# TimoLassmann/tagdust

Measured on AMD Instinct MI355X. Metric: reads/s (150 bp, 8-barcode arch), higher is better.
Workload: dtype f32

## Files before the change

tagdust_amd/csrc/td_jit.h:

```cpp
#pragma once
#include <string>
#include <vector>
#include "../../include/tagdust_hip.h"
#include "td_device.h"

#ifndef TD_HIDDEN
#define TD_HIDDEN __attribute__((visibility("hidden")))
#endif

struct TdSpecKnobs {
	int block = 512;
	int min_waves = 4;
	int lsum_oob = 1;
	int rt_min = 16;
	int groupcols = 18;
	int groupcols_fwd = 12;
	int prune = 1;
	int prune_sfx = 1;
	int restart = -1;
	int firstseg = -1;
	int trie_sh = 2;
	int profile = 0;
	int prune_stats = -1;
	std::string extra_opts;
};
TdSpecKnobs td_spec_knobs(void);

#define TD_PRUNE_TABLES 16
#define TD_PRUNE_RESTART_MAX 4

struct TdSpecPlan {
	TdSpecKnobs k;
	int S = 0, H = 0, C = 0;
	std::vector<int> col_off, hmm_off;
	std::vector<int> group, group_f;
	std::vector<int> pure_last, drop_m;
	std::vector<int> bw_off;
	int64_t halves = 0;
	std::vector<int> rt, rt_b;
	std::vector<int> base;
	std::vector<float> hi, lo, nv;
	bool trie_on = false;
	int trie_sh = 1, trie_n_share = 0;
	std::vector<int> trie_ord;
	int first_n = 0;
	int prune_segs = 0;
	int sfx_first = 0;
	float prune_z = 0.0f;
	int restart = 0;
};
TdSpecPlan td_spec_plan(const td_model_desc* m, const TdSpecKnobs& k);
TD_HIDDEN std::string td_spec_model_section(const td_model_desc* m, const TdSpecPlan& p, int lsum_oob, int window);

float td_spec_prune_z(const td_model_desc* m, int n_seg, int sfx_first);
void td_spec_prune_tables(const td_model_desc* m, const TdSpecPlan& p, int lcap, int stride, std::vector<float>& tab);
void td_spec_layout(TdSpecLayout& L, const TdSpecPlan& p, int lmax);
int td_spec_compile(const td_model_desc* m, const TdSpecPlan& p, int lsum_oob, int window, std::vector<char>& code, std::string& log,
                    uint64_t* key_out = nullptr, bool key_only = false);
int td_spec_compiles_started(void);
```

tagdust_amd/csrc/td_spec_kernel.inc:

```

#ifndef TDS_BLOCK
#define TDS_BLOCK 512
#endif
#ifndef TDS_MIN_WAVES
#define TDS_MIN_WAVES 4
#endif
#define TDS_REG_H 32
#define TDS_WPB (TDS_BLOCK / TD_WAVE)
#define NEG_INF (-__builtin_inff())
#define DEV __device__ __forceinline__

#define MODE_GET_LABEL 1
#define MODE_ARCH_COMP 5
#define OUT_SUCCESS 0
#define OUT_ARCH_MISMATCH 1
#define OUT_TOO_SHORT 2
#define OUT_BAR_FINGER_NOT_FOUND 3
#define OUT_MATCHES_ARTIFACTS 5
#define OUT_LOW_COMPLEXITY 6
#define N_OUTCOME_SLOTS 8
#define TDS_DIAG(k) (N_OUTCOME_SLOTS + 256 + ((k) - 192))

#ifndef TDS_LSUM_OOB
#define TDS_LSUM_OOB 1
// ... 127 lines not shown
DEV float emit_rt(const int b, const float hi, const float lo, const float nv, const BaseMask& k, const int x)
{
	const float r = (x == b) ? hi : lo;
	return k.m4 ? nv : r;
}

#ifndef TDS_PROFILE
#define TDS_PROFILE 0
#endif
#define TDS_PHASE(k) do { if (TDS_PROFILE) { const long long t_ = (long long)__builtin_readcyclecounter(); \
	if (lane == 0) atomicAdd(&ka.counters[TDS_DIAG(240 + (k))], (unsigned long long)(t_ - tprof)); tprof = t_; } } while (0)

#ifndef TDS_WINDOW
#define TDS_WINDOW 0
#endif
constexpr bool kMaskDP = TD_H - kFirstN <= TDS_REG_H;

struct Wv {
	uint32_t* pmask;
	int nwm;
	uint8_t* slot;
	int lane, len, lmax, tmax, tmin;
	float* bm;
	uint8_t* ba;
	int cut;
	int cutS;
	const float* wa;
	const float* wb;
	int sstop;
	int sstopS;
	const float* wc;
	const float* wd;
	mutable int bad;
	bool rb_on, rf_on;
	float* rs;
	float* hb;
	int rWf;
	int rW;
	const float* bwt;
	const float* fbs;
	unsigned long long* stats;
	long long* tprof;
	const float* ptab;
	int pstride;
	const float* qr;
	const float* pr;
};

#ifndef TDS_LATE_CS
#define TDS_LATE_CS 1
#endif
#ifndef TDS_PF_DIST
#define TDS_PF_DIST 4
#endif
#ifndef TDS_PF_COLS
#define TDS_PF_COLS 2
#endif
#ifndef TDS_LDP
#define TDS_LDP 2
#endif
#ifndef TDS_LDT
#define TDS_LDT 4
#endif
#ifndef TDS_SCAN_B
#define TDS_SCAN_B 8
#endif
#ifndef TDS_PRUNE_TT
#define TDS_PRUNE_TT (-88.0f)
#endif
#ifndef TDS_PRUNE_MARGIN
#define TDS_PRUNE_MARGIN 1
#endif
#ifndef TDS_PRUNE_BGAP
#define TDS_PRUNE_BGAP 5.0f
#endif
#ifndef TDS_PRUNE_STATS
#define TDS_PRUNE_STATS 0
#endif

constexpr int cmin(int a, int b) { return a < b ? a : b; }
constexpr int pf_dist(int cols, bool rt) { return (!rt && cols <= TDS_PF_COLS) ? TDS_PF_DIST : 1; }
template <int D> struct IC { static constexpr int v = D; };
constexpr bool label_leading(int h)
{
	for (int j = 0; j < kPruneSegs; j++) if (h >= kHmmOff[j] && h < kHmmOff[j] + kNHmm[j]) return true;
	return false;
}
template <int PD, int D, typename F>
DEV void ring_block(F& step, const int base)
{
	if constexpr (D < PD) { step(IC<D>{}, base + D); ring_block<PD, D + 1>(step, base); }
}
template <int PD, int D, typename F>
DEV void ring_rest(F& step, const int base, const int iend)
{
	if constexpr (D < PD - 1) { if (base + D <= iend) { step(IC<D>{}, base + D); ring_rest<PD, D + 1>(step, base, iend); } }
}

template <int J, bool RT>
DEV void bwd_row(const int fa, const float (&Mn)[kNCol[J]], const float (&In)[kNCol[J]], const float Pn,
                 const BaseMask& kc, const int c, const BaseMask& kx, const int xi, SV (&Mc)[kNCol[J]], SV (&Ic)[kNCol[J]])
{
#define EM(gcol, mask, xval) (RT ? emit_rt(kBase[colr + (gcol)], kHi[J], kLo[J], kNv[J], mask, xval) : EMIT_M(col0 + (gcol), mask))
	constexpr int NC = kNCol[J];
	constexpr int K = NC - 1;
	const int col0 = kColOff[J] + (RT ? 0 : fa) * NC;
// ... 631 lines not shown
	constexpr int NC = kNCol[J];
	float hi0 = NEG_INF;
	{
		const float* gf = w.ptab + (int64_t)(12 + J - kSfxFirst) * w.pstride;
		const int t = q_lo - 1;
		for (int k0 = 1; k0 <= t; k0 += 8) {
			float pr[8];
#pragma unroll
			for (int u = 0; u < 8; u++) { const int k = k0 + u; pr[u] = w.pr[((k <= t) ? t - k : 0) * TD_WAVE + w.lane]; }
			__builtin_amdgcn_sched_barrier(0);
#pragma unroll
			for (int u = 0; u < 8; u++) { const int k = k0 + u; if (k <= t) hi0 = fmaxf(hi0, uload(gf, k) + pr[u]); }
		}
		hi0 = fminf(hi0 + (__logf((float)(t > 1 ? t : 1)) + 0.02f), w.fbs[t]);
	}
	float Mlo[NC], Mhi[NC], Ilo[NC], Ihi[NC];
#pragma unroll
	for (int g = 0; g < NC; g++) { Mlo[g] = NEG_INF; Ilo[g] = NEG_INF; Mhi[g] = hi0; Ihi[g] = hi0; }
	int gc = 0;
	int closed_at = -1;
	auto close_check = [&](const int steps_done) __attribute__((always_inline)) {
		if (gc < NC) {
			bool cl = true;
#pragma unroll
			for (int g = 0; g < NC; g++) if (g == gc) cl = same(si(Mlo[g], Mhi[g])) && same(si(Ilo[g], Ihi[g]));
			if (__builtin_amdgcn_ballot_w64(!cl) == 0) { gc++; if (gc == NC) closed_at = steps_done; }
		}
	};
	int c_n = codes[q_lo * TD_WAVE + w.lane];
	float Pm_n = P[(q_lo - 1) * TD_WAVE + w.lane];
	for (int i = q_lo; i < q_hi; ++i) {
		const int c = c_n;
		const float Pm = Pm_n;
		{
			const int ip = (i + 1 < q_hi) ? i + 1 : i;
			c_n = codes[ip * TD_WAVE + w.lane];
			Pm_n = P[(ip - 1) * TD_WAVE + w.lane];
		}
		close_check(i - q_lo); close_check(i - q_lo);
		fstair_dispatch<J, 0>(gc, Mlo, Mhi, Ilo, Ihi, Pm, mk_mask(c));
	}
	close_check(q_hi - q_lo); close_check(q_hi - q_lo);
	if (gc < NC) w.bad |= 32;
	if (TDS_PRUNE_STATS && w.lane == 0) {
		const int st = closed_at >= 0 ? closed_at : q_hi - q_lo;
		atomicAdd(&w.stats[TDS_DIAG(194)], (unsigned long long)st); atomicAdd(&w.stats[TDS_DIAG(195)], 1ull);
		atomicMax(&w.stats[TDS_DIAG(192)], (unsigned long long)st);
	}
	float* rs = w.rs + (int64_t)kColOff[J] * 2 * TD_WAVE + w.lane;
#pragma unroll
	for (int g = 0; g < NC; g++) { rs[(2 * g) * TD_WAVE] = Mlo[g]; rs[(2 * g + 1) * TD_WAVE] = Ilo[g]; }
}

template <int J, int NF, bool RT>
DEV void fwd_group(const Wv& w, const uint8_t* __restrict__ codes, const float* __restrict__ P,
                   float* __restrict__ Cs, const float* __restrict__ PB, const uint8_t* __restrict__ BW,
                   float* __restrict__ DP, float* __restrict__ TOTAL, const float b, const int f0)
{
	const bool first = (f0 == 0);
#define EM(gcol, mask, xval) (RT ? emit_rt(kBase[colr + (gcol)], kHi[J], kLo[J], kNv[J], mask, xval) : EMIT_M(col0 + (gcol), mask))
	constexpr int NC = kNCol[J];
	constexpr int K = NC - 1;
	constexpr bool pure = kPureLast[J] != 0;
	constexpr int NS = NC - kPureLast[J];
	constexpr int DM = kDropM[J];
	constexpr int NSF = NS - DM;
	constexpr int ROWH = 2 * NS - DM;
	constexpr int NQ = NSF / 2;
	constexpr int NT = NSF & 1;
	constexpr bool skip_live = LIVE(kSkip[J]);
	float Mp[NF][NC], Ip[NF][NC], tot[NF];
#pragma unroll
	for (int f = 0; f < NF; f++) {
		tot[f] = NEG_INF;
#pragma unroll
		for (int g = 0; g < NC; g++) { Mp[f][g] = NEG_INF; Ip[f][g] = NEG_INF; }
	}
	if (TDS_RESTART && J >= kSfxFirst && w.rf_on) {
		const float* rs = w.rs + (int64_t)kColOff[J] * 2 * TD_WAVE + w.lane;
#pragma unroll
		for (int g = 0; g < NC; g++) { Mp[0][g] = rs[(2 * g) * TD_WAVE]; Ip[0][g] = rs[(2 * g + 1) * TD_WAVE]; }
	}
	constexpr bool p_init = (J == 0);
	const bool resumed = TDS_RESTART && (J >= kSfxFirst) && w.rf_on;
	const int i0 = resumed ? w.sstop - (TD_S - 1 - J) * (w.rWf + 1) : 1;
	float Pm = p_init ? 0.0f : P[(i0 - 1) * TD_WAVE + w.lane];
	constexpr int PD = pf_dist(NF * NC, RT);
	const int pmax = (w.tmax >= 1) ? w.tmax : 1;
	int c_q[PD];
	float Pi_q[PD], cs_q[PD], pb_q[PD], bm_q[PD], ik_q[PD][NF];
	int ba_q[PD];
	float MB_q[PD][NF][NSF + 1], IB_q[PD][NF][NSF + 1];
	constexpr bool pb_init = (J == TD_S - 1);
#define PBR(pos) (pb_init ? (((pos) == w.len + 1) ? 0.0f : NEG_INF) : PB[(pos) * TD_WAVE + w.lane])
#define BWROW(f_, pos_) (BW + ((int64_t)kBwOff[kHmmOff[J] + f0 + (f_)] * w.lmax + (int64_t)((pos_) - 1) * ROWH) * (TD_WAVE * 4))
#define TDS_FWD_FILL(d, p_raw) { \
		const int p_ = ((p_raw) <= pmax) ? (p_raw) : pmax; \
		c_q[d] = codes[p_ * TD_WAVE + w.lane]; \
		Pi_q[d] = p_init ? NEG_INF : P[p_ * TD_WAVE + w.lane]; \
		if (!first) cs_q[d] = Cs[p_ * TD_WAVE + w.lane]; \
		if (pure) pb_q[d] = PBR(p_ + 1); \
		if (own_sum && !first) { bm_q[d] = w.bm[p_ * TD_WAVE + w.lane]; ba_q[d] = w.ba[p_ * TD_WAVE + w.lane]; } \
		const bool rows_ = !((J >= kSfxFirst) && p_ < w.sstop);    \
_Pragma("unroll") \
		for (int f = 0; f < NF; f++) { \
			if (DM && rows_) ik_q[d][f] = ld1(BWROW(f, p_) + NSF * (TD_WAVE * 8), w.lane); \
			if (PD > 1 && rows_) { \
_Pragma("unroll") \
				for (int q = 0; q < NQ; q++) { \
					MB_q[d][f][2 * q] = ldk(BWROW(f, p_) + q * (TD_WAVE * 16), w.lane, 16, 0); IB_q[d][f][2 * q] = ldk(BWROW(f, p_) + q * (TD_WAVE * 16), w.lane, 16, 1); \
					MB_q[d][f][2 * q + 1] = ldk(BWROW(f, p_) + q * (TD_WAVE * 16), w.lane, 16, 2); IB_q[d][f][2 * q + 1] = ldk(BWROW(f, p_) + q * (TD_WAVE * 16), w.lane, 16, 3); \
				} \
				if (NT) { MB_q[d][f][NSF - 1] = ldk(BWROW(f, p_) + NQ * (TD_WAVE * 16), w.lane, 8, 0); IB_q[d][f][NSF - 1] = ldk(BWROW(f, p_) + NQ * (TD_WAVE * 16), w.lane, 8, 1); } \
			} \
		} \
	}
	constexpr bool own_sum = (J == 0) && (kFirstN > 0);
	float lacc[NF];
	uint32_t mbits[NF];
#pragma unroll
	for (int f = 0; f < NF; f++) { lacc[f] = 0.0f; mbits[f] = 0u; }
#pragma unroll
	for (int d = 0; d < PD; d++) {
		cs_q[d] = NEG_INF; pb_q[d] = 0.0f; bm_q[d] = -1.0f; ba_q[d] = 0;
#pragma unroll
		for (int f = 0; f < NF; f++) ik_q[d][f] = NEG_INF;
		TDS_FWD_FILL(d, i0 + d)
	}

	const int iend = (J < kPruneSegs && w.cut < w.tmax) ? w.cut : w.tmax;
	const int itail = (J == kPruneSegs && kPruneSegs > 0) ? w.cut + 1 : w.tmax + 1;
	(void)itail;
	if (i0 > 1 && kMaskDP && !own_sum) {
#pragma unroll
		for (int f = 0; f < NF; f++) {
			if (w.lane == 0) for (int wd = 0; wd < ((i0 - 1) >> 5); wd++) w.pmask[(kHmmOff[J] + f0 + f) * w.nwm + wd] = 0u;
			mbits[f] = 0u;
		}
	}
	auto step_cs = [&](auto dtag, auto cstag, const int i) __attribute__((always_inline)) {
		constexpr int d_ = decltype(dtag)::v;
		constexpr bool want_cs = decltype(cstag)::v != 0;
		const int c = c_q[d_];
		const float Pi = Pi_q[d_];
		const float pb = pb_q[d_];
		SV cs; cs.v = cs_q[d_]; cs.z = RT ? false : first;
		float bm = bm_q[d_];
		int ba = ba_q[d_];
		f32x4 cb[NF][NQ + 1];
		f32x2 ct[NF];
		const bool sfx_skip = (J >= kSfxFirst) && i < w.sstop;
		float ik[NF];
#pragma unroll
		for (int f = 0; f < NF; f++) {
			if constexpr (PD == 1) {
				const uint8_t* bw = BW + ((int64_t)kBwOff[kHmmOff[J] + f0 + f] * w.lmax + (int64_t)(i - 1) * ROWH) * (TD_WAVE * 4);
				if (!sfx_skip) {
#pragma unroll
					for (int p = 0; p < NQ; p++) cb[f][p] = ld4(bw + p * (TD_WAVE * 16), w.lane);
					if (NT) ct[f] = ld2(bw + NQ * (TD_WAVE * 16), w.lane);
				}
			} else {
#pragma unroll
				for (int p = 0; p < NQ; p++) cb[f][p] = f32x4{ MB_q[d_][f][2 * p], IB_q[d_][f][2 * p], MB_q[d_][f][2 * p + 1], IB_q[d_][f][2 * p + 1] };
				if (NT) ct[f] = f32x2{ MB_q[d_][f][NSF - 1], IB_q[d_][f][NSF - 1] };
			}
			ik[f] = ik_q[d_][f];
		}
		TDS_FWD_FILL(d_, i + PD)
		const int dn_ = (d_ + 1) % PD;
		const int c_n = c_q[dn_];
		const float pb_n = pb_q[dn_];
		float ik_n[NF];
#pragma unroll
		for (int f = 0; f < NF; f++) ik_n[f] = ik_q[dn_][f];
		float lpost[NF];
#pragma unroll
		for (int f = 0; f < NF; f++) lpost[f] = NEG_INF;
		const bool tail = (J == kPruneSegs && kPruneSegs > 0) && i >= itail;
		if (i <= w.len) {
			const SV PmS = sv(tail ? NEG_INF : Pm);
			const SV PiS = sv(tail ? NEG_INF : Pi);
			const BaseMask kc = mk_mask(c);
#pragma unroll
			for (int f = 0; f < NF; f++) {
				const int col0 = kColOff[J] + (RT ? 0 : (f0 + f)) * NC;
				const int colr = kColOff[J] + (f0 + f) * NC;
				(void)colr;
				const int h = kHmmOff[J] + f0 + f;
				SV Mc[NC], Ic[NC];
				SV Dc = sv_none();
				const float ei0 = EMIT_I(col0, kc);
				{
					const int q = col0;
					const SV M = addv(addc(PmS, kCols[q].sM), EM(0, kc, c));
					SV I = addc(PmS, kCols[q].sI);
					if (tail && LIVE(kCols[q].sI)) {
						if (!(Ip[f][0] + kCols[q].t[3] >= uload(w.wa, i))) w.bad |= 1;
					}
					I = lsum(I, addc(sv(Ip[f][0]), kCols[q].t[3]));
					I = lsum(I, addc(sv(Mp[f][0]), kCols[q].t[1]));
					I = addv(I, ei0);
					if (want_cs) { cs = lsum(cs, addc(M, kCols[q].t[7])); cs = lsum(cs, addc(I, kCols[q].t[8])); }
					Mc[0] = M; Ic[0] = I;
				}
#pragma unroll
				for (int g = 1; g <= K; ++g) {
					const int q = col0 + g, qp = q - 1;
					SV M = addc(PmS, kCols[q].sM);
					SV I = addc(PmS, kCols[q].sI);
					lsum2(M, addc(sv(Mp[f][g - 1]), kCols[qp].t[0]), I, addc(sv(Ip[f][g]), kCols[q].t[3]));
					lsum2(M, addc(sv(Ip[f][g - 1]), kCols[qp].t[4]), I, addc(sv(Mp[f][g]), kCols[q].t[1]));
					SV D = addc(Mc[g - 1], kCols[qp].t[2]);
					lsum2(M, addc(Dc, kCols[qp].t[6]), D, addc(Dc, kCols[qp].t[5]));
					M = addv(M, EM(g, kc, c));
					I = addv(I, EMIT_I(q, kc));
					if (want_cs) { cs = lsum(cs, addc(M, kCols[q].t[7])); cs = lsum(cs, addc(I, kCols[q].t[8])); }
					Mc[g] = M; Ic[g] = I; Dc = D;
				}
				if (tail && skip_live) { if (!(cs.v >= uload(w.wb, i))) w.bad |= 2; }
				if (want_cs) cs = lsum(cs, addc(PiS, kSkip[J]));
				if (!sfx_skip) {
				float MB[NC], IB[NC];
#pragma unroll
				for (int p = 0; p < NQ; p++) {
					const f32x4 v = cb[f][p];
					MB[2 * p] = v.x; IB[2 * p] = v.y; MB[2 * p + 1] = v.z; IB[2 * p + 1] = v.w;
				}
				if (NT) { MB[NSF - 1] = ct[f].x; IB[NSF - 1] = ct[f].y; }
				if constexpr (DM != 0) {
					constexpr int g = K - 1;
					const int q = col0 + g;
					const bool nxt = i < w.len;
					const int cx = (i < w.tmax) ? c_n : 0;
					const BaseMask kn = mk_mask(cx);
					SV MnK = addc(sv(pb_n), kCols[col0 + K].t[7]);
					if (!MnK.z) MnK.v = nxt ? MnK.v : NEG_INF;
					const float InK = nxt ? ik_n[f] : NEG_INF;
					SV Mr = addc(addv(MnK, EM(K, kn, cx)), kCols[q].t[0]);
					Mr = lsum(Mr, addc(sv(pb), kCols[q].t[7]));
					Mr = lsum(Mr, addc(addv(sv(InK), EMIT_I(q, kn)), kCols[q].t[1]));
					MB[g] = Mr.v; IB[g] = ik[f];
				}
				if (pure) {
					MB[K] = pb + kCols[col0 + K].t[7];
					IB[K] = pb + kCols[col0 + K].t[8];
				}
				constexpr bool want_tt = kNHmm[J] > 1;
				SV acc = sv_none(), tt = sv(tot[f]);
#pragma unroll
				for (int g = 0; g <= K; ++g) {
					const SV pm = subv(addv(Mc[g], MB[g]), b);
					if (want_tt && g == 0) tt = lsum(tt, pm);
					acc = lsum(acc, pm);
					if (want_tt && g == 0) tt = lsum(tt, subv(addv(addv(addc(PmS, kCols[col0].sI), ei0), IB[0]), b));
					acc = lsum(acc, subv(addv(Ic[g], IB[g]), b));
				}
				if (want_tt) tot[f] = tt.v;
				if (own_sum) {
					lacc[f] = post_prob(acc.v) + lacc[f];
					if (lacc[f] > bm) { bm = lacc[f]; ba = h; }
				} else if (kMaskDP) {
					lpost[f] = acc.v;
				} else {
					DP[((int64_t)(i - 1) * TD_H + h) * TD_WAVE + w.lane] = post_prob(acc.v);
				}
				}
#pragma unroll
				for (int g = 0; g < NC; g++) { Mp[f][g] = Mc[g].v; Ip[f][g] = Ic[g].v; }
			}
			if (want_cs) Cs[i * TD_WAVE + w.lane] = cs.v;
			if (own_sum) { w.bm[i * TD_WAVE + w.lane] = bm; w.ba[i * TD_WAVE + w.lane] = (uint8_t)ba; }
		}
		if (kMaskDP && !own_sum) {
#pragma unroll
			for (int f = 0; f < NF; f++) {
				const bool on = lpost[f] > -103.98f;
				const bool any_on = __builtin_amdgcn_ballot_w64(on) != 0;
				if (any_on) {
					float pp = 0.0f;
					if (on) pp = (float)exp((double)lpost[f]);
					if (i <= w.len) DP[((int64_t)(i - 1) * TD_H + kHmmOff[J] + f0 + f) * TD_WAVE + w.lane] = pp;
				}
				mbits[f] |= (any_on ? 1u : 0u) << ((i - 1) & 31);
				if ((((i - 1) & 31) == 31) || i == iend) {
					if (w.lane == 0) w.pmask[(kHmmOff[J] + f0 + f) * w.nwm + ((i - 1) >> 5)] = mbits[f];
					mbits[f] = 0u;
				}
			}
		}
		Pm = Pi;
	};
	{
		constexpr bool cs_late = TDS_LATE_CS && (J == TD_S - 1) && !((J == kPruneSegs && kPruneSegs > 0) && skip_live);
		auto step = [&](auto dtag, const int i) __attribute__((always_inline)) { step_cs(dtag, IC<1>{}, i); };
		auto step_nocs = [&](auto dtag, const int i) __attribute__((always_inline)) { step_cs(dtag, IC<0>{}, i); };
		int base = i0;
		if constexpr (cs_late) {
			const int i_cs = (w.tmin < iend) ? w.tmin : iend;
			for (; base + PD - 1 < i_cs; base += PD) ring_block<PD, 0>(step_nocs, base);
		}
		for (; base + PD - 1 <= iend; base += PD) ring_block<PD, 0>(step, base);
		ring_rest<PD, 0>(step, base, iend);
	}
	if (J < kPruneSegs && iend < w.tmax) {
		if (kMaskDP && !own_sum && w.lane == 0) {
#pragma unroll
			for (int f = 0; f < NF; f++)
				for (int wd = ((iend - 1) >> 5) + 1; wd < w.nwm; wd++) w.pmask[(kHmmOff[J] + f0 + f) * w.nwm + wd] = 0u;
		}
		if (kNHmm[J] > 1 && w.len > iend) {
#pragma unroll
			for (int f = 0; f < NF; f++) if (!(tot[f] >= TDS_PRUNE_TT)) w.bad |= 4;
		}
	}
	if (kNHmm[J] > 1) {
#pragma unroll
		for (int f = 0; f < NF; f++) TOTAL[(kHmmOff[J] + f0 + f) * TD_WAVE + w.lane] = tot[f];
	}
#undef EM
#undef PBR
#undef BWROW
#undef TDS_FWD_FILL
}

template <int J, int F0>
DEV void fwd_groups(const Wv& w, const uint8_t* __restrict__ codes, const float* __restrict__ P,
                    float* __restrict__ Cs, const float* __restrict__ PB, const uint8_t* __restrict__ BW,
                    float* __restrict__ DP, float* __restrict__ TOTAL, const float b)
{
	if constexpr (TDS_RESTART && F0 == 0 && J >= kSfxFirst) {
		if (w.rf_on) {
			const int q_hi = w.sstop - (TD_S - 1 - J) * (w.rWf + 1);
			fwd_stair<J>(w, codes, P, q_hi - w.rWf, q_hi);
		}
	}
	if constexpr (F0 == 0 && kRt[J] > 0) {
		for (int f0 = 0; f0 < kRt[J]; f0 += kGroupF[J]) fwd_group<J, kGroupF[J], true>(w, codes, P, Cs, PB, BW, DP, TOTAL, b, f0);
		fwd_groups<J, kRt[J]>(w, codes, P, Cs, PB, BW, DP, TOTAL, b);
	} else if constexpr (F0 < kNHmm[J]) {
		constexpr int NF = cmin(kGroupF[J], kNHmm[J] - F0);
		fwd_group<J, NF, false>(w, codes, P, Cs, PB, BW, DP, TOTAL, b, F0);
		fwd_groups<J, F0 + NF>(w, codes, P, Cs, PB, BW, DP, TOTAL, b);
	}
}

template <int J>
DEV void fwd_segments(const Wv& w, const uint8_t* __restrict__ codes, float* __restrict__ SF, const float* __restrict__ SB,
                      int rowlen, const uint8_t* __restrict__ BW, float* __restrict__ DP, float* __restrict__ TOTAL, const float b)
{
	if constexpr (J < TD_S) {
		fwd_groups<J, 0>(w, codes, SF + (int64_t)J * rowlen, SF + (int64_t)(J + 1) * rowlen, SB + (int64_t)(J + 1) * rowlen,
		                 BW, DP, TOTAL, b);
		if (TDS_PROFILE == 2 && J < 8) { const long long t_ = (long long)__builtin_readcyclecounter(); if (w.lane == 0) atomicAdd(&w.stats[TDS_DIAG(216 + J)], (unsigned long long)(t_ - *w.tprof)); *w.tprof = t_; }
		fwd_segments<J + 1>(w, codes, SF, SB, rowlen, BW, DP, TOTAL, b);
	}
}

constexpr bool path_word_trivial(int k)
{
	for (int b = 0; b < 4; b++) {
		const int v = kFirstN + 4 * k + b;
		if (v < TD_H && (kPredFirst[v] != 0 || kPredOff2[v + 1] != kPredOff2[v])) return false;
	}
	return true;
}
constexpr uint32_t path_word_identity(int k)
{
	uint32_t w = 0;
	for (int b = 0; b < 4; b++) w |= (uint32_t)((kFirstN + 4 * k + b) & 0xFF) << (8 * b);
	return w;
}

DEV int prune_scan(const float thr, const int len, const int tmax, const float* __restrict__ fbt, const float* __restrict__ bwt)
{
	int cl = 1;
	for (int i0 = 2; i0 <= tmax; i0 += TDS_SCAN_B) {
		float g[TDS_SCAN_B];
#pragma unroll
		for (int k = 0; k < TDS_SCAN_B; k++) {
			const int i = i0 + k;
			const int mm = (i <= len) ? len - i : 0;
			g[k] = bwt[mm];
		}
		__builtin_amdgcn_sched_barrier(0);
#pragma unroll
		for (int k = 0; k < TDS_SCAN_B; k++) g[k] = uload(fbt, i0 + k) + g[k];
#pragma unroll
		for (int k = 0; k < TDS_SCAN_B; k++) {
			const int i = i0 + k;
			if (i <= len && i <= tmax && g[k] > thr) cl = i;
		}
	}
#pragma unroll
	for (int o = 32; o >= 1; o >>= 1) cl = max(cl, __shfl_xor(cl, o));
	return __builtin_amdgcn_readfirstlane(cl);
}

DEV float leading_bwd_bound(const Wv& w, const int i)
{
	float hb = NEG_INF;
	for (int k0 = 0; i + 1 + k0 <= w.tmax + 1; k0 += TDS_SCAN_B) {
		float q[TDS_SCAN_B];
#pragma unroll
		for (int u = 0; u < TDS_SCAN_B; u++) {
// ... 905 lines not shown
```

tagdust_amd/csrc/td_spec_plan.cpp:

```cpp
#include <math.h>
#include <stdio.h>
#include <stdlib.h>
#include <string.h>

#include <map>
#include <string>
#include <vector>

#include "td_jit.h"

static std::string flit(float v)
{
	if (isinf(v)) return v < 0 ? "(-__builtin_inff())" : "__builtin_inff()";
	if (v != v) return "__builtin_nanf(\"\")";
	char buf[64];
	snprintf(buf, sizeof buf, "%af", (double)v);
	return buf;
}

TdSpecKnobs td_spec_knobs(void)
{
	TdSpecKnobs k;
	auto num = [](const char* name, int unset) { const char* e = getenv(name); return e ? atoi(e) : unset; };
	auto flag = [](const char* name, int unset) -> int { const char* e = getenv(name); return e ? atoi(e) != 0 : unset; };
	if (const int v = num("TD_SPEC_BLOCK", 0); v >= 64 && v <= 1024 && v % 64 == 0) k.block = v;
	if (const int v = num("TD_SPEC_MINWAVES", 0); v >= 1 && v <= 8) k.min_waves = v;
	if (const int v = num("TD_SPEC_GROUPCOLS", 0); v > 0) k.groupcols = v;
	k.groupcols_fwd = num("TD_SPEC_GROUPCOLS_FWD", k.groupcols_fwd);
	k.rt_min = num("TD_SPEC_RT_MIN", k.rt_min);
	k.trie_sh = num("TD_SPEC_TRIE_SH", k.trie_sh);
	k.profile = num("TD_SPEC_PROFILE", k.profile);
	k.lsum_oob = flag("TD_SPEC_LSUM_OOB", k.lsum_oob);
	k.prune = flag("TD_SPEC_PRUNE", k.prune);
	k.prune_sfx = flag("TD_SPEC_PRUNE_SFX", k.prune_sfx);
	k.restart = flag("TD_SPEC_RESTART", k.restart);
	k.firstseg = flag("TD_SPEC_FIRSTSEG", k.firstseg);
	k.prune_stats = flag("TD_SPEC_PRUNE_STATS", k.prune_stats);
	if (const char* e = getenv("TD_SPEC_EXTRA_OPTS")) k.extra_opts = e;
	return k;
}

namespace {
int pure_last(const td_model_desc* m, int j, int col_off)
{
	for (int f = 0; f < m->n_hmm[j]; f++) {
		const int q = col_off + f * m->n_col[j] + m->n_col[j] - 1;
		if (!(m->trans[q * 9 + 4] == -INFINITY) || !(m->trans[q * 9 + 3] == -INFINITY)) return 0;
	}
	return 1;
}

int rt_prefix(const td_model_desc* m, int j, int col_off, int* base , float* hi, float* lo, float* nv, int min_hmms)
{
	const int n = m->n_hmm[j], nc = m->n_col[j];
	if (n < min_hmms) return 0;
	auto match_type = [&](int q, int* b, float* h, float* l, float* v) -> bool {
		const float* e = m->eM + (size_t)q * 5;
		for (int x = 0; x < 4; x++) {
			const float other = e[(x + 1) & 3];
			bool ok = !(e[x] == other);
			for (int y = 0; y < 4 && ok; y++) if (y != x && !(e[y] == other)) ok = false;
			if (ok) { *b = x; *h = e[x]; *l = other; *v = e[4]; return true; }
		}
		return false;
	};
	int b0; float h0, l0, v0;
	if (!match_type(col_off, &b0, &h0, &l0, &v0)) return 0;
	int f = 0;
	for (; f < n; f++) {
		bool ok = true;
		for (int g = 0; g < nc && ok; g++) {
			const int q = col_off + f * nc + g, q0 = col_off + g;
			if (memcmp(m->trans + (size_t)q * 9, m->trans + (size_t)q0 * 9, 36) || memcmp(m->eI + (size_t)q * 5, m->eI + (size_t)q0 * 5, 20) ||
			    memcmp(&m->sM[q], &m->sM[q0], 4) || memcmp(&m->sI[q], &m->sI[q0], 4)) { ok = false; break; }
			int b; float h, l, v;
			if (!match_type(q, &b, &h, &l, &v) || memcmp(&h, &h0, 4) || memcmp(&l, &l0, 4) || memcmp(&v, &v0, 4)) { ok = false; break; }
			base[q] = b;
		}
		if (!ok) break;
	}
	*hi = h0; *lo = l0; *nv = v0;
	return f >= min_hmms ? f : 0;
}

int group_size(int n_hmm, int n_col, int target)
{
	int maxf = target / n_col;
	if (maxf < 1) maxf = 1;
	if (maxf > n_hmm) maxf = n_hmm;
	const int groups = (n_hmm + maxf - 1) / maxf;
	return (n_hmm + groups - 1) / groups;
}

int first_labels(const td_model_desc* m, int firstseg)
{
	const int H = m->H, n0 = m->n_hmm[0];
	const int mode = firstseg >= 0 ? firstseg : H > 32;
	if (!mode) return 0;
	if (n0 < 2 || n0 >= H) return 0;
	for (int v = 0; v < n0; v++)
		for (int u = 0; u < v; u++) if (m->A[u * H + v] == 1.0f) return 0;
	for (int w = n0; w < H; w++) {
		int c = 0;
		for (int u = 0; u < n0; u++) c += m->A[u * H + w] == 1.0f;
		if (c != 0 && c != n0) return 0;
	}
	return n0;
}

bool read_like(const td_model_desc* m, int j, int co)
{
	if (m->n_hmm[j] != 1 || m->n_col[j] != 1) return false;
	const float* t = m->trans + (size_t)co * 9;
	for (int k = 0; k < 9; k++) if (k != TD_II && k != TD_ISKIP && t[k] > -INFINITY) return false;
	return m->sM[co] == -INFINITY && m->sI[co] > -INFINITY && t[TD_II] > -INFINITY && t[TD_ISKIP] > -INFINITY;
}
}

TdSpecPlan td_spec_plan(const td_model_desc* m, const TdSpecKnobs& k)
{
	TdSpecPlan p;
	const int S = m->S, H = m->H, C = m->C;
	p.k = k; p.S = S; p.H = H; p.C = C;
	p.col_off.resize(S); p.hmm_off.resize(S);
	for (int j = 0, co = 0, ho = 0; j < S; co += m->n_hmm[j] * m->n_col[j], ho += m->n_hmm[j], j++) { p.col_off[j] = co; p.hmm_off[j] = ho; }
	p.group.resize(S); p.group_f.resize(S); p.pure_last.resize(S); p.drop_m.resize(S); p.bw_off.resize(H);
	for (int j = 0; j < S; j++) {
		p.group[j] = group_size(m->n_hmm[j], m->n_col[j], k.groupcols);
		p.group_f[j] = group_size(m->n_hmm[j], m->n_col[j], k.groupcols_fwd > 0 ? k.groupcols_fwd : k.groupcols);
		p.pure_last[j] = pure_last(m, j, p.col_off[j]);
	}
	int cols = 0;
	for (int j = 0; j < S; j++) {
		p.drop_m[j] = m->n_col[j] >= 2 && p.pure_last[j];
		for (int f = 0; f < m->n_hmm[j]; f++) { p.bw_off[p.hmm_off[j] + f] = cols; cols += 2 * (m->n_col[j] - p.pure_last[j]) - p.drop_m[j]; }
	}
	p.halves = cols;
	p.rt.assign(S, 0); p.rt_b.assign(S, 0); p.base.assign(C, 0);
	p.hi.assign(S, 0.0f); p.lo.assign(S, 0.0f); p.nv.assign(S, 0.0f);
	for (int j = 0; j < S; j++) {
		const int pre = rt_prefix(m, j, p.col_off[j], p.base.data(), &p.hi[j], &p.lo[j], &p.nv[j], k.rt_min);
		if (pre > 0) {
			p.group_f[j] = p.group[j];
			p.rt[j] = pre / p.group[j] * p.group[j];
			p.rt_b[j] = p.rt[j];
		} else {
			p.rt_b[j] = rt_prefix(m, j, p.col_off[j], p.base.data(), &p.hi[j], &p.lo[j], &p.nv[j], 2);
		}
	}
	{
		const int sh = k.trie_sh;
		bool on = p.rt[0] > 0 && sh >= 1 && m->n_col[0] >= sh + 2;
		std::vector<int> ord;
		int n_share = 0;
		if (on) {
			const int G = p.group[0], NC0 = m->n_col[0];
			std::map<std::vector<int>, std::vector<int>> cls;
			for (int f = 0; f < p.rt[0]; f++) {
				std::vector<int> key;
				for (int g = NC0 - sh; g < NC0; g++) key.push_back(p.base[(size_t)(p.col_off[0] + f * NC0 + g)]);
				cls[key].push_back(f);
			}
			std::vector<int> left;
			for (auto& kv : cls) {
				const std::vector<int>& v = kv.second;
				const size_t full = v.size() / (size_t)G * (size_t)G;
				for (size_t i = 0; i < full; i++) ord.push_back(v[i]);
				for (size_t i = full; i < v.size(); i++) left.push_back(v[i]);
			}
			n_share = (int)ord.size() / G;
			for (int f : left) ord.push_back(f);
			if (n_share == 0) on = false;
		}
		if (!on) { ord.assign(1, 0); n_share = 0; }
		p.trie_on = on; p.trie_sh = on ? sh : 1; p.trie_n_share = n_share; p.trie_ord = ord;
	}
	p.first_n = first_labels(m, k.firstseg);
	p.prune_segs = 0; p.sfx_first = S;
	if (k.prune && H - p.first_n <= 32) {
		int first = -1, last = -1;
		for (int j = 0; j < S; j++) if (read_like(m, j, p.col_off[j])) { if (first < 0) first = j; last = j; }
		if (first > 0) p.prune_segs = first;
		bool single = k.prune_sfx && last >= 0 && last < S - 1;
		for (int j = last + 1; single && j < S; j++) if (m->n_hmm[j] != 1) single = false;
		if (single) p.sfx_first = last + 1;
	}
	p.prune_z = td_spec_prune_z(m, p.prune_segs, p.sfx_first);
	if (p.prune_segs <= 0 || p.prune_segs > TD_PRUNE_RESTART_MAX || (p.sfx_first < S && S - p.sfx_first > TD_PRUNE_RESTART_MAX)) p.restart = 0;
	else if (k.restart >= 0) p.restart = k.restart;
	else p.restart = p.col_off[p.prune_segs] >= 48;
	return p;
}

std::string td_spec_model_section(const td_model_desc* m, const TdSpecPlan& p, int lsum_oob, int window)
{
	std::string s;
	char buf[256];
	const int S = m->S, H = m->H, C = m->C;
	int req = 0;
	for (int j = 0; j < S; j++) if (m->seg_type[j] == 'F') req += m->finger_len[j];
	snprintf(buf, sizeof buf, "#define TDS_BLOCK %d\n#define TDS_MIN_WAVES %d\n", p.k.block, p.k.min_waves);
	s += buf;
	snprintf(buf, sizeof buf, "#define TDS_LSUM_OOB %d\n", lsum_oob != 0);
	s += buf;
	snprintf(buf, sizeof buf, "#define TDS_WINDOW %d\n", window != 0);
	s += buf;
	snprintf(buf, sizeof buf, "#define TDS_PROFILE %d\n", p.k.profile);
	s += buf;
	snprintf(buf, sizeof buf, "#define TD_S %d\n#define TD_H %d\n#define TD_C %d\n#define TD_REQ_FINGER %d\n", S, H, C, req);
	s += buf;
	s += "struct GCol { float t[9]; float sM, sI; float eM[5]; float eI[5]; };\n";
	auto int_array = [&](const char* name, const std::vector<int>& v) {
		s += std::string("static constexpr int ") + name + "[" + std::to_string(v.size()) + "] = {";
		for (size_t i = 0; i < v.size(); i++) { s += std::to_string(v[i]); if (i + 1 < v.size()) s += ","; }
		s += "};\n";
	};
	int_array("kNHmm", std::vector<int>(m->n_hmm, m->n_hmm + S)); int_array("kNCol", std::vector<int>(m->n_col, m->n_col + S));
	int_array("kColOff", p.col_off); int_array("kHmmOff", p.hmm_off);
	int_array("kRtB", p.rt_b);
	s += std::string("static constexpr bool kTrieOn = ") + (p.trie_on ? "true" : "false") + ";\n";
	s += "static constexpr int kTrieSH = " + std::to_string(p.trie_sh) + ";\n";
	s += "static constexpr int kTrieNShare = " + std::to_string(p.trie_n_share) + ";\n";
	int_array("kTrieOrd", p.trie_ord);
	int_array("kGroup", p.group); int_array("kGroupF", p.group_f); int_array("kPureLast", p.pure_last); int_array("kDropM", p.drop_m); int_array("kBwOff", p.bw_off);
	int_array("kRt", p.rt); int_array("kBase", p.base);
	auto float_array = [&](const char* name, const std::vector<float>& v) {
		s += std::string("static constexpr float ") + name + "[" + std::to_string(v.size()) + "] = {";
		for (size_t i = 0; i < v.size(); i++) { s += flit(v[i]); if (i + 1 < v.size()) s += ","; }
		s += "};\n";
	};
	float_array("kHi", p.hi); float_array("kLo", p.lo); float_array("kNv", p.nv);
	s += "static constexpr float kSkip[" + std::to_string(S) + "] = {";
	for (int j = 0; j < S; j++) { s += flit(m->skip[j]); if (j + 1 < S) s += ","; }
	s += "};\n";
	s += "static constexpr float kBg[5] = {";
	for (int i = 0; i < 5; i++) { s += flit(m->bg[i]); if (i < 4) s += ","; }
	s += "};\n";
	const float stay_arg = (float)(1.0 - (1.0 / (double)(float)m->avg_len));
	const float exit_arg = (float)(1.0 / (double)(float)m->avg_len);
	s += "static constexpr float kRStay = " + flit(stay_arg == 0.0f ? -INFINITY : (float)log((double)stay_arg)) + ";\n";
	s += "static constexpr float kRExit = " + flit(exit_arg == 0.0f ? -INFINITY : (float)log((double)exit_arg)) + ";\n";
	s += "static constexpr GCol kCols[" + std::to_string(C) + "] = {\n";
	for (int k = 0; k < C; k++) {
		s += " {{";
		for (int t = 0; t < 9; t++) { s += flit(m->trans[k * 9 + t]); if (t < 8) s += ","; }
		s += "}," + flit(m->sM[k]) + "," + flit(m->sI[k]) + ",{";
		for (int e = 0; e < 5; e++) { s += flit(m->eM[k * 5 + e]); if (e < 4) s += ","; }
		s += "},{";
		for (int e = 0; e < 5; e++) { s += flit(m->eI[k * 5 + e]); if (e < 4) s += ","; }
		s += "}},\n";
	}
	s += "};\n";
	s += "static constexpr unsigned kHinfo[" + std::to_string(H) + "] = {";
	for (int h = 0; h < H; h++) {
		const int seg = m->label[h] & 0xFFFF, f = (m->label[h] >> 16) & 0x7FFF;
		unsigned v = (unsigned)(unsigned char)m->seg_type[seg] | ((unsigned)seg << 8) | ((unsigned)f << 16);
		if (m->seg_type[seg] == 'B' && f == m->n_hmm[seg] - 1) v |= 0x80000000u;
		snprintf(buf, sizeof buf, "0x%08xu%s", v, h + 1 < H ? "," : "");
		s += buf;
	}
	s += "};\n";
	std::vector<int> poff(H + 1, 0), pidx;
	for (int v = 0; v < H; v++) {
		poff[v] = (int)pidx.size();
		for (int u = 0; u < v; u++) if (m->A[u * H + v] == 1.0f) pidx.push_back(u);
	}
	poff[H] = (int)pidx.size();
	if (pidx.empty()) pidx.push_back(0);
	int_array("kPredOff", poff); int_array("kPredIdx", pidx);
	const int first_n = p.first_n;
	std::vector<int> pfirst(H, 0), poff2(H + 1, 0), pidx2;
	for (int v = 0; v < H; v++) {
		poff2[v] = (int)pidx2.size();
		for (int i = poff[v]; i < poff[v + 1]; i++) {
			if (pidx[i] < first_n) pfirst[v] = 1; else pidx2.push_back(pidx[i]);
		}
	}
// ... 40 lines not shown
```

Measured before the change: 83.14 million.

## Share identical prefix columns across HMMs in forward groups and prefetch rows ahead

The planner now groups non-runtime-template HMMs in the forward pass by how many leading columns they share with an earlier HMM in the same group. The kernel copies those shared M/I/D states from the donor HMM instead of recomputing them, using compile-time donor tables emitted into the JIT source. It also issues the backward-row loads for the next HMM while the current one computes, when groups hold three or more HMMs. The aim is to cut redundant forward DP arithmetic and hide load latency. The cost is larger unrolled code and register arrays that hold all per-group states at once, which may raise register pressure.

```diff
diff --git a/tagdust_amd/csrc/td_jit.h b/tagdust_amd/csrc/td_jit.h
--- a/tagdust_amd/csrc/td_jit.h
+++ b/tagdust_amd/csrc/td_jit.h
@@ -15,6 +15,8 @@
 	int rt_min = 16;
 	int groupcols = 18;
 	int groupcols_fwd = 12;
+	int fwd_share = 1;
+	int fwd_hmms = 3;
 	int prune = 1;
 	int prune_sfx = 1;
 	int restart = -1;
@@ -34,6 +36,7 @@
 	int S = 0, H = 0, C = 0;
 	std::vector<int> col_off, hmm_off;
 	std::vector<int> group, group_f;
+	std::vector<int> fwd_grp_off, fwd_grp_start, fwd_grp_size, fwd_don;
 	std::vector<int> pure_last, drop_m;
 	std::vector<int> bw_off;
 	int64_t halves = 0;
diff --git a/tagdust_amd/csrc/td_spec_kernel.inc b/tagdust_amd/csrc/td_spec_kernel.inc
--- a/tagdust_amd/csrc/td_spec_kernel.inc
+++ b/tagdust_amd/csrc/td_spec_kernel.inc
@@ -203,6 +203,9 @@
 #endif
 #ifndef TDS_PF_DIST
 #define TDS_PF_DIST 4
+#endif
+#ifndef TDS_FWD_ROWS_AHEAD
+#define TDS_FWD_ROWS_AHEAD 1
 #endif
 #ifndef TDS_PF_COLS
 #define TDS_PF_COLS 2
@@ -940,7 +943,18 @@
 	for (int g = 0; g < NC; g++) { rs[(2 * g) * TD_WAVE] = Mlo[g]; rs[(2 * g + 1) * TD_WAVE] = Ilo[g]; }
 }
 
-template <int J, int NF, bool RT>
+template <int I, int N, typename F>
+DEV void each_ic(F&& fn)
+{
+	if constexpr (I < N) { fn(IC<I>{}); each_ic<I + 1, N>(fn); }
+}
+template <int J, int F0, bool RT>
+constexpr int fwd_src(int f, int g)
+{
+	return RT ? f : kFwdDon[kColOff[J] + (F0 + f) * kNCol[J] + g] - F0;
+}
+
+template <int J, int NF, bool RT, int F0S>
 DEV void fwd_group(const Wv& w, const uint8_t* __restrict__ codes, const float* __restrict__ P,
                    float* __restrict__ Cs, const float* __restrict__ PB, const uint8_t* __restrict__ BW,
                    float* __restrict__ DP, float* __restrict__ TOTAL, const float b, const int f0)
@@ -1039,15 +1053,19 @@
 		f32x2 ct[NF];
 		const bool sfx_skip = (J >= kSfxFirst) && i < w.sstop;
 		float ik[NF];
+		constexpr bool rows_ahead = TDS_FWD_ROWS_AHEAD && PD == 1 && NF >= 3;
+		auto load_rows = [&](const int f) __attribute__((always_inline)) {
+			const uint8_t* bw = BW + ((int64_t)kBwOff[kHmmOff[J] + f0 + f] * w.lmax + (int64_t)(i - 1) * ROWH) * (TD_WAVE * 4);
+			if (!sfx_skip) {
+#pragma unroll
+				for (int p = 0; p < NQ; p++) cb[f][p] = ld4(bw + p * (TD_WAVE * 16), w.lane);
+				if (NT) ct[f] = ld2(bw + NQ * (TD_WAVE * 16), w.lane);
+			}
+		};
 #pragma unroll
 		for (int f = 0; f < NF; f++) {
 			if constexpr (PD == 1) {
-				const uint8_t* bw = BW + ((int64_t)kBwOff[kHmmOff[J] + f0 + f] * w.lmax + (int64_t)(i - 1) * ROWH) * (TD_WAVE * 4);
-				if (!sfx_skip) {
-#pragma unroll
-					for (int p = 0; p < NQ; p++) cb[f][p] = ld4(bw + p * (TD_WAVE * 16), w.lane);
-					if (NT) ct[f] = ld2(bw + NQ * (TD_WAVE * 16), w.lane);
-				}
+				if (!rows_ahead || f == 0) load_rows(f);
 			} else {
 #pragma unroll
 				for (int p = 0; p < NQ; p++) cb[f][p] = f32x4{ MB_q[d_][f][2 * p], IB_q[d_][f][2 * p], MB_q[d_][f][2 * p + 1], IB_q[d_][f][2 * p + 1] };
@@ -1070,42 +1088,57 @@
 			const SV PmS = sv(tail ? NEG_INF : Pm);
 			const SV PiS = sv(tail ? NEG_INF : Pi);
 			const BaseMask kc = mk_mask(c);
-#pragma unroll
-			for (int f = 0; f < NF; f++) {
+			SV Mn[NF][NC], In[NF][NC], Dn[NF][NC];
+			each_ic<0, NF>([&](auto ftag) __attribute__((always_inline)) {
+				constexpr int f = decltype(ftag)::v;
 				const int col0 = kColOff[J] + (RT ? 0 : (f0 + f)) * NC;
 				const int colr = kColOff[J] + (f0 + f) * NC;
 				(void)colr;
 				const int h = kHmmOff[J] + f0 + f;
-				SV Mc[NC], Ic[NC];
-				SV Dc = sv_none();
+				SV (&Mc)[NC] = Mn[f];
+				SV (&Ic)[NC] = In[f];
+				if constexpr (rows_ahead && f + 1 < NF) load_rows(f + 1);
 				const float ei0 = EMIT_I(col0, kc);
 				{
 					const int q = col0;
-					const SV M = addv(addc(PmS, kCols[q].sM), EM(0, kc, c));
-					SV I = addc(PmS, kCols[q].sI);
-					if (tail && LIVE(kCols[q].sI)) {
-						if (!(Ip[f][0] + kCols[q].t[3] >= uload(w.wa, i))) w.bad |= 1;
+					constexpr int s0 = fwd_src<J, F0S, RT>(f, 0);
+					if constexpr (s0 != f) {
+						Mc[0] = Mn[s0][0]; Ic[0] = In[s0][0];
+					} else {
+						const SV M = addv(addc(PmS, kCols[q].sM), EM(0, kc, c));
+						SV I = addc(PmS, kCols[q].sI);
+						if (tail && LIVE(kCols[q].sI)) {
+							if (!(Ip[f][0] + kCols[q].t[3] >= uload(w.wa, i))) w.bad |= 1;
+						}
+						I = lsum(I, addc(sv(Ip[f][0]), kCols[q].t[3]));
+						I = lsum(I, addc(sv(Mp[f][0]), kCols[q].t[1]));
+						I = addv(I, ei0);
+						Mc[0] = M; Ic[0] = I;
 					}
-					I = lsum(I, addc(sv(Ip[f][0]), kCols[q].t[3]));
-					I = lsum(I, addc(sv(Mp[f][0]), kCols[q].t[1]));
-					I = addv(I, ei0);
-					if (want_cs) { cs = lsum(cs, addc(M, kCols[q].t[7])); cs = lsum(cs, addc(I, kCols[q].t[8])); }
-					Mc[0] = M; Ic[0] = I;
-				}
-#pragma unroll
-				for (int g = 1; g <= K; ++g) {
+					Dn[f][0] = sv_none();
+					if (want_cs) { cs = lsum(cs, addc(Mc[0], kCols[q].t[7])); cs = lsum(cs, addc(Ic[0], kCols[q].t[8])); }
+				}
+				each_ic<1, NC>([&](auto gtag) __attribute__((always_inline)) {
+					constexpr int f = decltype(ftag)::v;
+					constexpr int g = decltype(gtag)::v;
 					const int q = col0 + g, qp = q - 1;
-					SV M = addc(PmS, kCols[q].sM);
-					SV I = addc(PmS, kCols[q].sI);
-					lsum2(M, addc(sv(Mp[f][g - 1]), kCols[qp].t[0]), I, addc(sv(Ip[f][g]), kCols[q].t[3]));
-					lsum2(M, addc(sv(Ip[f][g - 1]), kCols[qp].t[4]), I, addc(sv(Mp[f][g]), kCols[q].t[1]));
-					SV D = addc(Mc[g - 1], kCols[qp].t[2]);
-					lsum2(M, addc(Dc, kCols[qp].t[6]), D, addc(Dc, kCols[qp].t[5]));
-					M = addv(M, EM(g, kc, c));
-					I = addv(I, EMIT_I(q, kc));
-					if (want_cs) { cs = lsum(cs, addc(M, kCols[q].t[7])); cs = lsum(cs, addc(I, kCols[q].t[8])); }
-					Mc[g] = M; Ic[g] = I; Dc = D;
-				}
+					constexpr int s = fwd_src<J, F0S, RT>(f, g);
+					if constexpr (s != f) {
+						Mn[f][g] = Mn[s][g]; In[f][g] = In[s][g]; Dn[f][g] = Dn[s][g];
+					} else {
+						constexpr int sp = fwd_src<J, F0S, RT>(f, g - 1);
+						SV M = addc(PmS, kCols[q].sM);
+						SV I = addc(PmS, kCols[q].sI);
+						lsum2(M, addc(sv(Mp[sp][g - 1]), kCols[qp].t[0]), I, addc(sv(Ip[f][g]), kCols[q].t[3]));
+						lsum2(M, addc(sv(Ip[sp][g - 1]), kCols[qp].t[4]), I, addc(sv(Mp[f][g]), kCols[q].t[1]));
+						SV D = addc(Mn[f][g - 1], kCols[qp].t[2]);
+						lsum2(M, addc(Dn[f][g - 1], kCols[qp].t[6]), D, addc(Dn[f][g - 1], kCols[qp].t[5]));
+						M = addv(M, EM(g, kc, c));
+						I = addv(I, EMIT_I(q, kc));
+						Mn[f][g] = M; In[f][g] = I; Dn[f][g] = D;
+					}
+					if (want_cs) { cs = lsum(cs, addc(Mn[f][g], kCols[q].t[7])); cs = lsum(cs, addc(In[f][g], kCols[q].t[8])); }
+				});
 				if (tail && skip_live) { if (!(cs.v >= uload(w.wb, i))) w.bad |= 2; }
 				if (want_cs) cs = lsum(cs, addc(PiS, kSkip[J]));
 				if (!sfx_skip) {
@@ -1154,8 +1187,11 @@
 					DP[((int64_t)(i - 1) * TD_H + h) * TD_WAVE + w.lane] = post_prob(acc.v);
 				}
 				}
-#pragma unroll
-				for (int g = 0; g < NC; g++) { Mp[f][g] = Mc[g].v; Ip[f][g] = Ic[g].v; }
+			});
+#pragma unroll
+			for (int f = 0; f < NF; f++) {
+#pragma unroll
+				for (int g = 0; g < NC; g++) if (fwd_src<J, F0S, RT>(f, g) == f) { Mp[f][g] = Mn[f][g].v; Ip[f][g] = In[f][g].v; }
 			}
 			if (want_cs) Cs[i * TD_WAVE + w.lane] = cs.v;
 			if (own_sum) { w.bm[i * TD_WAVE + w.lane] = bm; w.ba[i * TD_WAVE + w.lane] = (uint8_t)ba; }
@@ -1212,24 +1248,24 @@
 #undef TDS_FWD_FILL
 }
 
-template <int J, int F0>
+template <int J, int GI, bool RTDONE = false>
 DEV void fwd_groups(const Wv& w, const uint8_t* __restrict__ codes, const float* __restrict__ P,
                     float* __restrict__ Cs, const float* __restrict__ PB, const uint8_t* __restrict__ BW,
                     float* __restrict__ DP, float* __restrict__ TOTAL, const float b)
 {
-	if constexpr (TDS_RESTART && F0 == 0 && J >= kSfxFirst) {
+	if constexpr (TDS_RESTART && !RTDONE && GI == kFwdGrpOff[J] && J >= kSfxFirst) {
 		if (w.rf_on) {
 			const int q_hi = w.sstop - (TD_S - 1 - J) * (w.rWf + 1);
 			fwd_stair<J>(w, codes, P, q_hi - w.rWf, q_hi);
 		}
 	}
-	if constexpr (F0 == 0 && kRt[J] > 0) {
-		for (int f0 = 0; f0 < kRt[J]; f0 += kGroupF[J]) fwd_group<J, kGroupF[J], true>(w, codes, P, Cs, PB, BW, DP, TOTAL, b, f0);
-		fwd_groups<J, kRt[J]>(w, codes, P, Cs, PB, BW, DP, TOTAL, b);
-	} else if constexpr (F0 < kNHmm[J]) {
-		constexpr int NF = cmin(kGroupF[J], kNHmm[J] - F0);
-		fwd_group<J, NF, false>(w, codes, P, Cs, PB, BW, DP, TOTAL, b, F0);
-		fwd_groups<J, F0 + NF>(w, codes, P, Cs, PB, BW, DP, TOTAL, b);
+	if constexpr (!RTDONE && GI == kFwdGrpOff[J] && kRt[J] > 0) {
+		for (int f0 = 0; f0 < kRt[J]; f0 += kGroupF[J]) fwd_group<J, kGroupF[J], true, 0>(w, codes, P, Cs, PB, BW, DP, TOTAL, b, f0);
+		fwd_groups<J, GI, true>(w, codes, P, Cs, PB, BW, DP, TOTAL, b);
+	} else if constexpr (GI < kFwdGrpOff[J + 1]) {
+		constexpr int F0 = kFwdGrpStart[GI], NF = kFwdGrpSize[GI];
+		fwd_group<J, NF, false, F0>(w, codes, P, Cs, PB, BW, DP, TOTAL, b, F0);
+		fwd_groups<J, GI + 1, true>(w, codes, P, Cs, PB, BW, DP, TOTAL, b);
 	}
 }
 
@@ -1238,7 +1274,7 @@
                       int rowlen, const uint8_t* __restrict__ BW, float* __restrict__ DP, float* __restrict__ TOTAL, const float b)
 {
 	if constexpr (J < TD_S) {
-		fwd_groups<J, 0>(w, codes, SF + (int64_t)J * rowlen, SF + (int64_t)(J + 1) * rowlen, SB + (int64_t)(J + 1) * rowlen,
+		fwd_groups<J, kFwdGrpOff[J]>(w, codes, SF + (int64_t)J * rowlen, SF + (int64_t)(J + 1) * rowlen, SB + (int64_t)(J + 1) * rowlen,
 		                 BW, DP, TOTAL, b);
 		if (TDS_PROFILE == 2 && J < 8) { const long long t_ = (long long)__builtin_readcyclecounter(); if (w.lane == 0) atomicAdd(&w.stats[TDS_DIAG(216 + J)], (unsigned long long)(t_ - *w.tprof)); *w.tprof = t_; }
 		fwd_segments<J + 1>(w, codes, SF, SB, rowlen, BW, DP, TOTAL, b);
diff --git a/tagdust_amd/csrc/td_spec_plan.cpp b/tagdust_amd/csrc/td_spec_plan.cpp
--- a/tagdust_amd/csrc/td_spec_plan.cpp
+++ b/tagdust_amd/csrc/td_spec_plan.cpp
@@ -27,6 +27,8 @@
 	if (const int v = num("TD_SPEC_MINWAVES", 0); v >= 1 && v <= 8) k.min_waves = v;
 	if (const int v = num("TD_SPEC_GROUPCOLS", 0); v > 0) k.groupcols = v;
 	k.groupcols_fwd = num("TD_SPEC_GROUPCOLS_FWD", k.groupcols_fwd);
+	k.fwd_share = flag("TD_SPEC_FWD_SHARE", k.fwd_share);
+	if (const int v = num("TD_SPEC_FWD_HMMS", 0); v >= 1) k.fwd_hmms = v;
 	k.rt_min = num("TD_SPEC_RT_MIN", k.rt_min);
 	k.trie_sh = num("TD_SPEC_TRIE_SH", k.trie_sh);
 	k.profile = num("TD_SPEC_PROFILE", k.profile);
@@ -92,6 +94,17 @@
 	return (n_hmm + groups - 1) / groups;
 }
 
+int shared_cols(const td_model_desc* m, int co, int nc, int f, int e)
+{
+	int g = 0;
+	for (; g < nc; g++) {
+		const size_t q = (size_t)(co + f * nc + g), r = (size_t)(co + e * nc + g);
+		if (memcmp(m->trans + q * 9, m->trans + r * 9, 36) || memcmp(&m->sM[q], &m->sM[r], 4) || memcmp(&m->sI[q], &m->sI[r], 4) ||
+		    memcmp(m->eM + q * 5, m->eM + r * 5, 20) || memcmp(m->eI + q * 5, m->eI + r * 5, 20)) break;
+	}
+	return g;
+}
+
 int first_labels(const td_model_desc* m, int firstseg)
 {
 	const int H = m->H, n0 = m->n_hmm[0];
@@ -148,6 +161,33 @@
 			p.rt_b[j] = rt_prefix(m, j, p.col_off[j], p.base.data(), &p.hi[j], &p.lo[j], &p.nv[j], 2);
 		}
 	}
+	p.fwd_grp_off.assign(S + 1, 0); p.fwd_grp_start.clear(); p.fwd_grp_size.clear(); p.fwd_don.assign(C, 0);
+	for (int j = 0; j < S; j++) {
+		const int n = m->n_hmm[j], nc = m->n_col[j], co = p.col_off[j];
+		p.fwd_grp_off[j] = (int)p.fwd_grp_start.size();
+		for (int f = 0; f < n; f++) for (int g = 0; g < nc; g++) p.fwd_don[co + f * nc + g] = f;
+		int f = p.rt[j];
+		if (p.rt[j] > 0 || !k.fwd_share) {
+			for (; f < n; f += p.group_f[j]) { p.fwd_grp_start.push_back(f); p.fwd_grp_size.push_back(n - f < p.group_f[j] ? n - f : p.group_f[j]); }
+			continue;
+		}
+		const int budget = k.groupcols_fwd > 0 ? k.groupcols_fwd : k.groupcols;
+		const int cap = k.fwd_hmms > p.group_f[j] ? k.fwd_hmms : p.group_f[j];
+		while (f < n) {
+			const int start = f;
+			int distinct = 0;
+			for (; f < n; f++) {
+				int best = 0;
+				for (int e = start; e < f; e++) { const int sh = shared_cols(m, co, nc, f, e); if (sh > best) best = sh; }
+				if (f > start && (distinct + nc - best > budget || f - start >= cap)) break;
+				distinct += nc - best;
+				for (int g = 0; g < best; g++)
+					for (int e = start; e < f; e++) if (shared_cols(m, co, nc, f, e) > g) { p.fwd_don[co + f * nc + g] = e; break; }
+			}
+			p.fwd_grp_start.push_back(start); p.fwd_grp_size.push_back(f - start);
+		}
+	}
+	p.fwd_grp_off[S] = (int)p.fwd_grp_start.size();
 	{
 		const int sh = k.trie_sh;
 		bool on = p.rt[0] > 0 && sh >= 1 && m->n_col[0] >= sh + 2;
@@ -223,6 +263,11 @@
 	s += "static constexpr int kTrieNShare = " + std::to_string(p.trie_n_share) + ";\n";
 	int_array("kTrieOrd", p.trie_ord);
 	int_array("kGroup", p.group); int_array("kGroupF", p.group_f); int_array("kPureLast", p.pure_last); int_array("kDropM", p.drop_m); int_array("kBwOff", p.bw_off);
+	{
+		std::vector<int> gs = p.fwd_grp_start, gn = p.fwd_grp_size;
+		if (gs.empty()) { gs.push_back(0); gn.push_back(0); }
+		int_array("kFwdGrpOff", p.fwd_grp_off); int_array("kFwdGrpStart", gs); int_array("kFwdGrpSize", gn); int_array("kFwdDon", p.fwd_don);
+	}
 	int_array("kRt", p.rt); int_array("kBase", p.base);
 	auto float_array = [&](const char* name, const std::vector<float>& v) {
 		s += std::string("static constexpr float ") + name + "[" + std::to_string(v.size()) + "] = {";
```

Result: no change. 83.88 million, median of 6 (+0.9%).
